# ducha-aiki/mods-light-zmq

Measured on AMD Instinct MI355X. Metric: image_pairs_per_sec_end_to_end, higher is better.
Workload: dtype f32

## Files before the change

### include/mods_hip.h

```cpp
#ifndef MODS_HIP_H
#define MODS_HIP_H

#include <stddef.h>
#include <stdint.h>

#ifdef __cplusplus
extern "C" {
#endif

#define MODS_OK 0
#define MODS_E_NODEVICE (-1)
#define MODS_E_ARG (-2)
#define MODS_E_CAPACITY (-3)
#define MODS_E_HIP (-4)

typedef struct mods_ctx mods_ctx;

typedef struct mods_hessaff_params {
  int numberOfScales;
  float initialSigma;
  float threshold;
  float edgeEigenValueRatio;
  int border;
  int maxIterations;
// ... 54 lines not shown
void *mods_ctx_stream(mods_ctx *ctx);

enum { MODS_STAGE_BLUR = 0, MODS_STAGE_RESPONSE, MODS_STAGE_RESIZE, MODS_STAGE_NMS, MODS_STAGE_LOCALIZE,
       MODS_STAGE_BAUMBERG, MODS_STAGE_SORT, MODS_STAGE_ORIENT, MODS_STAGE_DESCRIBE, MODS_STAGE_MATCH,
       MODS_STAGE_RANSAC_SCORE, MODS_STAGE_SYNTH,
       MODS_STAGE_BLUR_SMALL,
       MODS_STAGE_PYRAMID,
       MODS_STAGE_MATCH_NN1,
       MODS_STAGE_EXTRACT,
       MODS_STAGE_SIFT,
       MODS_STAGE_GUIDED,
       MODS_STAGE_MATCH_MUTUAL,
       MODS_STAGE_OVERLAP,
       MODS_STAGE_OVERLAP_AREA,
       MODS_STAGE_LOCAL_AFFINE,
       MODS_STAGE_REPROJECT_H,
       MODS_STAGE_COUNT };
int mods_ctx_timing_enable(mods_ctx *ctx, int stage_mask);
int mods_ctx_graphs(mods_ctx *ctx, int on);
long mods_ctx_graph_replays(const mods_ctx *ctx);
long mods_ctx_u8_source_calls(const mods_ctx *ctx);
int mods_ctx_u8_kernels(mods_ctx *ctx, int mask);
long mods_ctx_u8_strip_calls(const mods_ctx *ctx);
int mods_u8_strips_layout(int w, int h, unsigned *max_width, unsigned *n_strips, unsigned *pitch, size_t *image_bytes);
void mods_u8_strips_strip_of(unsigned n, unsigned *out);
int mods_u8_strips_offsets(int w, int h, unsigned *out);
int mods_u8_strips_fetch(mods_ctx *ctx, const unsigned char *img_u8_host, int n_img, int w, int h, int src_offset, unsigned char *out);
int mods_ctx_pyramid_streams(mods_ctx *ctx, int n);
int mods_ctx_timing_read(mods_ctx *ctx, int stage, double *total_ms, int *launches, double *bytes);
int mods_ctx_timing_reset(mods_ctx *ctx);

int mods_detect_hessian_affine(mods_ctx *ctx, const float *img, int w, int h, int stride,
                               const mods_hessaff_params *par, mods_affkey *out, int max_out, int *n_out);
int mods_detect_hessian_affine_dev(mods_ctx *ctx, const float *img_dev, int n_img, int w, int h, int stride,
                                   const mods_hessaff_params *par, mods_affkey *out_host, int max_out,
                                   int *n_out_host);

int mods_pyramid_octaves(mods_ctx *ctx);
int mods_pyramid_dims(mods_ctx *ctx, int octave, int *w, int *h);
int mods_pyramid_plane(mods_ctx *ctx, int img, int octave, int level, int kind, float *dst_host);
int mods_pyramid_candidates(mods_ctx *ctx, int img, mods_candidate *out, int max_out, int *n_out);
int mods_pyramid_nms_hits(mods_ctx *ctx, int img, int *out4, int max_out, int *n_out);

int mods_gauss_blur(mods_ctx *ctx, const float *src, int w, int h, float sigma, float *dst);
int mods_hessian_response(mods_ctx *ctx, const float *src, int w, int h, float norm, float *dst);
int mods_resize_half(mods_ctx *ctx, const float *src, int w, int h, float *dst, int *dw, int *dh);
// ... 450 lines not shown
```

### mods-light-zmq_amd/__init__.py

```python
import ctypes as C
import os
import subprocess

import numpy as np

PKG_DIR = os.path.dirname(os.path.abspath(__file__))
LIB_PATH = os.environ.get("MODS_LIB") or os.path.join(PKG_DIR, "libmodsgpu.so")

MODS_OK = 0
STAGES = ["blur", "response", "resize", "nms", "localize", "baumberg", "sort", "orient", "describe", "match",
          "ransac_score", "synth", "blur_small", "pyramid", "match_nn1", "extract", "sift", "guided", "match_mutual",
          "overlap", "overlap_area"]
STAGES_LATER = ["local_affine", "reproject_h"]


def stage_index(name):
    return STAGES.index(name) if name in STAGES else len(STAGES) + STAGES_LATER.index(name)


class ModsError(RuntimeError):
    pass


class HessAffParams(C.Structure):
# ... 92 lines not shown
    return out[:n.value].copy(), u6[:n.value].copy(), laf[:n.value].copy()


def _overlap(fn, dtype, lists, params, cap):
    out = np.zeros(max(cap, 1), dtype)
    n = C.c_int()
    counts = OverlapCounts()
    _check(fn(*lists, C.byref(params), _vp(out), cap, C.byref(n), C.byref(counts)))
    return out[:n.value].copy(), counts


def _mask_rows(mask):
    m = np.asarray(mask)
    if m.dtype != np.uint8 or m.ndim != 2 or m.size == 0:
        raise ValueError("a detection mask is a non-empty 2-D uint8 array")
    if m.strides[1] != 1 or m.strides[0] < m.shape[1]:
        m = np.ascontiguousarray(m)
    return m, m.strides[0]


def detection_mask_test(mask, x, y):
    m, stride = _mask_rows(mask)
    return bool(lib().mods_detection_mask_test(_vp(m), m.shape[1], m.shape[0], stride, C.c_double(x), C.c_double(y)))


def u8_strips_layout(w, h):
    lim, ns, pitch, nbytes = C.c_uint(), C.c_uint(), C.c_uint(), C.c_size_t()
    _check(lib().mods_u8_strips_layout(int(w), int(h), C.byref(lim), C.byref(ns), C.byref(pitch), C.byref(nbytes)))
    return lim.value, ns.value, pitch.value, nbytes.value


def u8_strips_strip_of(n):
    out = np.zeros(int(n), np.uint32)
    lib().mods_u8_strips_strip_of(C.c_uint(int(n)), C.c_void_p(out.ctypes.data))
    return out


def u8_strips_offsets(w, h):
    out = np.zeros((int(h) - 1, int(w) - 1), np.uint32)
    _check(lib().mods_u8_strips_offsets(int(w), int(h), C.c_void_p(out.ctypes.data)))
    return out


class ViewGeom(C.Structure):
    _fields_ = [("identity", C.c_int), ("w_rot", C.c_int), ("h_rot", C.c_int), ("w_new", C.c_int), ("h_new", C.c_int),
                ("ksize_x", C.c_int), ("ksize_y", C.c_int), ("pad", C.c_int),
# ... 298 lines not shown
        out = np.zeros(max_out, REGION_DTYPE)
        n = C.c_int()
        _check(lib().mods_orient_describe_u8(self.h, C.c_void_p(a.ctypes.data), a.shape[1], a.shape[0], a.strides[0],
                                             k.ctypes.data_as(C.c_void_p), len(k), C.byref(params), out.ctypes.data_as(C.c_void_p),
                                             max_out, C.byref(n)))
        return out[:n.value].copy()

    def regions_fetch_half(self, img=0, max_out=1 << 18):
        out = np.zeros(max_out, REGION_DTYPE)
        n = C.c_int()
        _check(lib().mods_regions_fetch_half(self.h, img, out.ctypes.data_as(C.c_void_p), max_out, C.byref(n)))
        return out[:n.value].copy()

    def detect_describe_dev(self, dev_ptr, n_img, w, h, det=None, desc=None):
        det = det or HessAffParams.default()
        desc = desc or DescribeParams.default()
        nd, nr = (C.c_int * n_img)(), (C.c_int * n_img)()
        _check(lib().mods_detect_describe_dev(self.h, C.c_void_p(dev_ptr), n_img, w, h, w, C.byref(det), C.byref(desc), nd, nr))
        return list(nd), list(nr)

    def u8_source_calls(self):
        lib().mods_ctx_u8_source_calls.restype = C.c_long
        return int(lib().mods_ctx_u8_source_calls(self.h))

    def set_u8_kernels(self, mask):
        _check(lib().mods_ctx_u8_kernels(self.h, int(mask)))

    def u8_strip_calls(self):
        lib().mods_ctx_u8_strip_calls.restype = C.c_long
        return int(lib().mods_ctx_u8_strip_calls(self.h))

    def u8_strips_fetch(self, batch_u8, src_offset=0):
        a = np.ascontiguousarray(batch_u8, np.uint8)
        n, h, w = a.shape
        _, ns, pitch, nbytes = u8_strips_layout(w, h)
        out = np.zeros(n * nbytes, np.uint8)
        _check(lib().mods_u8_strips_fetch(self.h, C.c_void_p(a.ctypes.data), n, w, h, int(src_offset), C.c_void_p(out.ctypes.data)))
        return out.reshape(n, ns, pitch // 16, 16)

    def set_match_mutual(self, mode):
        _check(lib().mods_ctx_match_mutual(self.h, int(mode)))

    def set_local_affine(self, params=None):
        _check(lib().mods_ctx_local_affine(self.h, C.byref(params) if params is not None else None))

    def local_affine_counts(self):
# ... 1180 lines not shown
```

### mods-light-zmq_amd/csrc/capi.hip

```cpp
#include "common.hpp"
#include "u8_strips.hpp"
#include "detmath.hpp"
#include "ransac_host.hpp"
#include "f_laf.hpp"
#include "h_laf.hpp"
#include "../../include/mods_degensac.h"
#include <cstdarg>
#include <memory>
#include <algorithm>
#include <cmath>
#include <mutex>
#include <vector>
#include <time.h>
#include <sys/prctl.h>

namespace mods {

static thread_local char g_err[512] = "";

void set_error(const char *fmt, ...) {
  va_list ap;
  va_start(ap, fmt);
  vsnprintf(g_err, sizeof(g_err), fmt, ap);
  va_end(ap);
// ... 421 lines not shown
    c->dd_cache.emplace_back(key, ex);
    MODS_HIP_CHECK(hipGraphLaunch(ex, c->stream));
    c->dd_replays++;
    return MODS_OK;
  }
  if (g) (void)hipGraphDestroy(g);
  (void)hipGetLastError();
  c->pyr_side = false;
  c->dd_graphs = false;
  c->omap_dirty = true;
  return dd_enqueue(c, img, n_img, w, h, stride, det, desc);
}

int mods_ctx_graphs(mods_ctx *c, int on) {
  if (!c) return MODS_E_ARG;
  c->dd_graphs = on != 0;
  if (!on) { dd_graph_drop(c); c->dd_linear.clear(); }
  mods::dev_state_changed(c);
  return MODS_OK;
}
long mods_ctx_graph_replays(const mods_ctx *c) { return c ? c->dd_replays : 0; }
long mods_ctx_u8_source_calls(const mods_ctx *c) { return c ? c->u8_source_calls : 0; }
long mods_ctx_u8_strip_calls(const mods_ctx *c) { return c ? c->u8_strip_calls : 0; }
int mods_ctx_u8_kernels(mods_ctx *c, int mask) {
  if (!c || mask > 255) { set_error("u8_kernels: bad argument"); return MODS_E_ARG; }
  c->u8_kernels = mask < 0 ? -1 : mask;
  mods::dev_state_changed(c);
  return MODS_OK;
}

static int dd_call(mods_ctx *c, const PixelSources &img, int n_img, int w, int h, int stride, const mods_hessaff_params *det,
                   const mods_describe_params *desc, int *n_detected_host, int *n_regions_host) {
  int rc;
  if ((rc = mods::dsp_check(c, desc))) return rc;
  if ((rc = dd_run(c, img, n_img, w, h, stride, det, desc))) return rc;
  int *hc = c->host_counts;
  MODS_HIP_CHECK(mods::stream_wait(c->stream));
  for (int b = 0; b < n_img; b++) {
    if (hc[b] > c->max_cand) { set_error("NMS hit list overflow: %d > %d", hc[b], c->max_cand); return MODS_E_CAPACITY; }
    if (n_detected_host) n_detected_host[b] = hc[2 * c->batch + b];
    if (hc[3 * c->batch + b] > std::min(c->max_cand, 1 << 17)) { set_error("region list overflow: %d", hc[3 * c->batch + b]); return MODS_E_CAPACITY; }
    if (n_regions_host) n_regions_host[b] = hc[3 * c->batch + b];
  }
  c->last_region_counts.assign(hc + 3 * c->batch, hc + 3 * c->batch + n_img);
  c->last_inside_counts.assign(hc + 4 * c->batch, hc + 4 * c->batch + n_img);
  if (hc[5 * c->batch]) {
// ... 778 lines not shown
```

### mods-light-zmq_amd/csrc/common.hpp

```cpp
#pragma once
#include <hip/hip_runtime.h>
#include <atomic>
#include <chrono>
#include <cmath>
#include <cstdint>
#include <cstdio>
#include <cstring>
#include <string>
#include <vector>
#include "../../include/mods_hip.h"
#include "buffer.hpp"
#include "pixel_sources.hpp"
#include "detection_mask.hpp"

namespace mods {

void set_error(const char *fmt, ...);

#define MODS_HIP_CHECK(expr)                                                              \
  do {                                                                                    \
    hipError_t _e = (expr);                                                               \
    if (_e != hipSuccess) {                                                               \
      mods::set_error("%s failed: %s (%s:%d)", #expr, hipGetErrorString(_e), __FILE__, __LINE__); \
      return MODS_E_HIP;                                                                  \
// ... 163 lines not shown
  mods::Buf<int> cand_count;
  mods::Buf<mods_affkey> keys_dev;
  mods::Buf<unsigned long long> sort_keys;
  mods::Buf<int> sort_idx;
  mods::Buf<int> rank_dev;
  mods::Buf<unsigned long long> nms_mask;
  mods::PinnedBuf<int> host_counts;
  mods::Buf<unsigned char> u8_stage_dev;
  mods::Buf<unsigned char> u8_strip_dev;
  long u8_strip_calls = 0;
  int u8_kernels = -1;
  long u8_source_calls = 0;
  mods::Buf<unsigned char> clahe_lut;
  bool clahe_on = false;
  mods_clahe_params clahe_par = {0.0, 0, 0};
  mods::PinnedBuf<char> pin_arena;
  mods_hessaff_params par;
  int reg_number_eff = -1;
  int last_w = 0, last_h = 0, last_n_img = 0;
  const float *last_img_dev = nullptr; int last_stride = 0;
  mods::Buf<float> desc_tables_dev;
  mods::Buf<int> desc_err_dev;
  int desc_ori_ps = 0, desc_ps = 0;
  mods::Buf<char> ori_dev;
  mods::Buf<char> ori_multi_dev;
  mods::Buf<mods_region> regions_dev;
  mods::Buf<mods_region> regions_half_dev;
  bool have_half = false;
  mods::Buf<int> region_count;
  mods::Buf<int> inside_count;
  std::vector<int> last_inside_counts;
  mods::Buf<float> desc_scratch;
  int dsp_scales = 0;
  double dsp_start = 0, dsp_end = 0;
  mods::Buf<double> dsp_acc;
  int blur_table_ps = 0;
  mods::Buf<float> blur_table_dev;
  mods_descriptor_fn ext_fn = nullptr;
  void *ext_user = nullptr;
  double ext_mr = 0;
  int ext_ps = 0;
  mods_descriptor_fn shape_fn = nullptr, ori_fn = nullptr;
  void *shape_user = nullptr, *ori_user = nullptr;
  double shape_mr = 0, ori_mr = 0;
  int shape_ps = 0, ori_ps = 0;
  mods_net *shape_net = nullptr, *ori_net = nullptr, *ext_net = nullptr;
// ... 157 lines not shown
__host__ __device__ inline int la_len(int n, int max_n) { return n < 0 || n > max_n ? 0 : n; }
int la_check(const mods_local_affine_params *p, LaConst *k);
int la_reserve(mods_ctx *c, int n_jobs, int grid_n);
int la_filter_dev(mods_ctx *c, const LaJob *jobs, int n_jobs, int grid_n, const LaConst &k, const int **diag_counters = nullptr,
                  const int **diag_slots = nullptr, int *diag_stride = nullptr);
struct TentList;
int local_affine_prefilter(mods_ctx *c, const mods_pair_params *par, TentList *list, bool deduped);
static_assert(LA_MAX_JOBS >= kCountSlots - 1, "every pair of a batch has its slots in la_count");
int launch_fast_sqrt_selftest(mods_ctx *ctx, unsigned long long *out5_host);
int launch_blur_table(mods_ctx *ctx, int ps);
bool ransac_profile_on();
int ransac_profile_mode();

int describe_run(mods_ctx *ctx, const PixelSources &img, int n_img, int w, int h, const mods_describe_params *par);
int u8_to_f32_launch(mods_ctx *c, const unsigned char *src, int n_img, int w, int h, int stride, float *dst, bool strips = false);
int u8_sources_launch(mods_ctx *c, const unsigned char *src, int n_img, int w, int h, int stride, bool twin, PixelSources *img);
int u8_stage_ensure(mods_ctx *c);
int describe_run_view(mods_ctx *ctx, const PixelSources &img, int n_img, int w, int h, const mods_describe_params *par, const double *H,
                      int orig_w, int orig_h, mods_region *det_copy_dev);
bool view_region_frame(const double *H, int w, int h, int orig_w, int orig_h, DetGateFrame *frame);
int describe_configure(mods_ctx *ctx, const mods_describe_params *par);
int launch_dominant_angle_test(mods_ctx *ctx, const float *patch_dev, int ps, double th, float *out_dev);
int launch_sift_patch_test(mods_ctx *ctx, const float *patch_dev, int ps, int root, double max_bin, uint8_t *out_dev);
int launch_sift_pooled_test(mods_ctx *ctx, const float *patches_dev, int K, int ps, int root, int half, int photo, double max_bin,
                            uint8_t *out_dev);
int dsp_check(mods_ctx *ctx, const mods_describe_params *par);

inline bool has_hooks(const mods_ctx *c) { return c->ext_fn || c->shape_fn || c->ori_fn; }
inline bool has_nets(const mods_ctx *c) { return c->ext_net || c->shape_net || c->ori_net; }
int net_run_to_host(mods_ctx *ctx, mods_net *net, const float *patches_dev, int n, int quantise_u8, float *out_host);

int pair_gpu_stage(mods_ctx *c, const float *img_dev, int w, int h, int stride, const mods_pair_params *par, mods_pair_result *res,
                   TentList *list);
int pairs_gpu_stage(mods_ctx *c, const void *const *img, const int *kinds, int n_pairs, int w, int h, const mods_pair_params *par,
                    mods_pair_result *const *res, TentList *const *lists, const unsigned char *const *masks = nullptr);
int pair_verify_stage(int device, const mods_pair_params *par, mods_pair_result *res, TentList *list, double *matches_out,
                      int max_matches, int w, int h);

}

extern "C" {
int mods_match_copy_out(mods_ctx *c, int n, mods_tentative *tent, double *u6, double *laf);
int mods_match_fetch_internal(mods_ctx *c, mods_tentative *out, double *u6_out, double *laf_out, int max_out, int *n_out);
int mods_ransac_warmup(int device, int len);
int mods_ctx_warmup(mods_ctx *c, int n_img, int w, int h, const mods_pair_params *par);
}
// ... 1 lines not shown
```

### mods-light-zmq_amd/csrc/describe.hip

```cpp
#include "describe_common.hpp"
#include "detmath.hpp"
#include "device_util.hpp"

namespace mods {

struct OriOut { double a11, a12, a21, a22; int alive; int pad; };

__device__ unsigned char g_ori_bin[2048];
__global__ __launch_bounds__(256) void ori_bin_table_kernel() {
  const float PIf = 3.14159265358979323846f;
  const int bins = 36;
  const int e = blockIdx.x * 256 + threadIdx.x;
  const float ori = atan2_lut_case(e >> 8, g_atan_lut[e & 255]);
  g_ori_bin[e] = (unsigned char)(int)(bins * (ori / PIf + 1.0f) / 2.0f);
}

__device__ __forceinline__ float peak_angle(const float *s_hist, int b) {
  const int bins = 36;
  const float PIf = 3.14159265358979323846f;
  const int a = b == 0 ? bins - 1 : b - 1, c = b == bins - 1 ? 0 : b + 1;
  const float ha = s_hist[a], hb = s_hist[b], hc = s_hist[c];
  const float pp = (ha - hc) / (ha - 2.0f * hb + hc) / 2.0f;
  return 2.0f * PIf * (b + 0.5f + pp) / bins - PIf;
}
// ... 421 lines not shown
      !(par->desc_patchSize & 1)) { set_error("unsupported patch sizes (ori %d, desc %d)", par->ori_patchSize, par->desc_patchSize); return MODS_E_ARG; }
  if (!ctx->desc_tables_dev) {
    MODS_HIP_CHECK(mods::reserve_group(ctx->desc_tables_dev, kTabSift + (sizeof(SiftTab) + sizeof(float) - 1) / sizeof(float), ctx->desc_err_dev, 1));
    MODS_HIP_CHECK(hipMemsetAsync(ctx->desc_err_dev, 0, sizeof(int), ctx->stream));
  }
  if (ctx->desc_ori_ps != par->ori_patchSize || ctx->desc_ps != par->desc_patchSize) {
    std::vector<float> m1((size_t)64 * 64, 0.f), m2((size_t)64 * 64, 0.f);
    circular_gauss_mask_host(par->ori_patchSize, par->ori_patchSize / 3.0f, m1.data());
    circular_gauss_mask_host(par->desc_patchSize, 0.f, m2.data());
    SiftTab tab;
    build_sift_tab(par->desc_patchSize, &tab);
    mods::dev_state_changed(ctx);
    MODS_HIP_CHECK(mods::stream_wait(ctx->stream));
    MODS_HIP_CHECK(mods::copy_wait(ctx->stream, ctx->desc_tables_dev, m1.data(), sizeof(float) * 4096, hipMemcpyHostToDevice));
    MODS_HIP_CHECK(mods::copy_wait(ctx->stream, ctx->desc_tables_dev + kTabDescMask, m2.data(), sizeof(float) * 4096, hipMemcpyHostToDevice));
    {
      const int ps = par->ori_patchSize;
      std::vector<float> vm((size_t)64 * 64, 0.f);
      for (int p = 0; p < ps * (ps - 2); p++) { const int c = p % ps; vm[p] = (c >= 1 && c < ps - 1) ? m1[p + ps] : 0.f; }
      MODS_HIP_CHECK(mods::copy_wait(ctx->stream, ctx->desc_tables_dev + kTabVoteMask, vm.data(), sizeof(float) * 4096, hipMemcpyHostToDevice));
    }
    MODS_HIP_CHECK(mods::copy_wait(ctx->stream, ctx->desc_tables_dev + kTabSift, &tab, sizeof(SiftTab), hipMemcpyHostToDevice));
    ctx->desc_ori_ps = par->ori_patchSize; ctx->desc_ps = par->desc_patchSize;
  }
  return MODS_OK;
}

int describe_run(mods_ctx *ctx, const PixelSources &img, int n_img, int w, int h, const mods_describe_params *par) {
  return describe_run_view(ctx, img, n_img, w, h, par, nullptr, 0, 0, nullptr);
}

static int external_describe(mods_ctx *ctx, int n_img, const DescConst &k) {
  const int pp = k.desc_ps * k.desc_ps;
  std::vector<int> counts(n_img);
  MODS_HIP_CHECK(hipMemcpyAsync(counts.data(), ctx->region_count, sizeof(int) * n_img, hipMemcpyDeviceToHost, ctx->stream));
  MODS_HIP_CHECK(mods::stream_wait(ctx->stream));
  std::vector<float> patches, out;
  std::vector<uint8_t> desc;
  for (int b = 0; b < n_img; b++) {
    const int n = std::min(counts[b], k.reg_cap);
    if (n <= 0) continue;
    out.assign((size_t)n * 128, 0.f); desc.resize((size_t)n * 128);
    if (ctx->ext_net) {
      const int rc = net_run_to_host(ctx, ctx->ext_net, ctx->desc_scratch + (size_t)b * k.reg_cap * pp, n, ctx->ext_q8, out.data());
      if (rc) return rc;
    } else {
// ... 316 lines not shown
```

### mods-light-zmq_amd/csrc/sift.hip

```cpp
#include "describe_common.hpp"
#include "detmath.hpp"
#include "device_util.hpp"

namespace mods {

constexpr int SMALL_CAP = 80;
#ifndef EXTRACT_T_LO
#define EXTRACT_T_LO 48
#endif
#ifndef EXTRACT_T_MID
#define EXTRACT_T_MID 64
#endif
#ifndef ES_MINB
#define ES_MINB 5
#endif

__device__ __forceinline__ double *lds_doubles(float *base, const void *p) {
  const int off = (int)((const float *)p - base);
  return (double *)(base + ((off + 1) & ~1));
}

struct RegionGeom {
  int P2;
  float scale;
// ... 1055 lines not shown
      sift_tail(s_vec, s_sq, s_red, k.root != 0, k.max_bin, o + (size_t)b * img_stride + (size_t)ri * reg_stride, half != 0);
    }
  }
}

constexpr int SW_R = 8;
constexpr int SW_G = 68;
constexpr int SW_CW = 18;
constexpr int S2_MAX_IMG = 64;
constexpr int S2_WAVES = 12;
constexpr int S2_BINS = 1024;
__device__ __forceinline__ int s2_bin(int g, int br, int bc) { return (g >> 2) * 64 + br * 16 + (g & 3) * 4 + bc; }
__device__ __forceinline__ int s2_vec(int g, int i) { return (i & 7) * 128 + s2_bin(g, i >> 5, (i >> 3) & 3); }

__host__ __device__ constexpr int s2_row_slots(int ps) { return SW_R * ps + SW_CW + 2 > SW_R * SW_G / 2 ? SW_R * ps + SW_CW + 2 : SW_R * SW_G / 2; }
static size_t sift_wave2_wave_bytes(int ps) {
  return sizeof(double) * S2_BINS + sizeof(float2) * (size_t)s2_row_slots(ps) + sizeof(float) * 3 * SW_R;
}
static size_t sift_wave2_lds_bytes(int ps) {
  const size_t ppa = ((size_t)ps * ps + 7) & ~(size_t)7;
  return sizeof(float) * 2048 + sizeof(float) * (4 * ps + 4) + sizeof(int) * 72 + sizeof(unsigned short) * ppa + S2_WAVES * sift_wave2_wave_bytes(ps) + 64;
}

template <int NC, bool POOL = false>
__global__ __launch_bounds__(64 * S2_WAVES, 3) void sift_wave2_kernel(DescConst k, const float *__restrict__ patches, mods_region *__restrict__ reg_all,
                                                                        const int *__restrict__ reg_count, const float *__restrict__ mask,
                                                                        const SiftTab *__restrict__ tab, int n_img, int *__restrict__ next_unit,
                                                                        double *__restrict__ pool, int pool_first) {
  extern __shared__ __attribute__((aligned(16))) float smem[];
  const int ps = k.desc_ps, pp = ps * ps, ppa = (pp + 7) & ~7;
  const int tid = threadIdx.x, lane = tid & 63, wv = tid >> 6;
  float *s_ot = smem;
  float *s_w = s_ot + 2048;
  int *s_pref = (int *)(s_w + 4 * ps + 4);
  unsigned short *s_midx = (unsigned short *)(s_pref + 72);
  unsigned char *wbase = (unsigned char *)(s_midx + ppa) + (size_t)wv * (sizeof(double) * S2_BINS + sizeof(float2) * s2_row_slots(ps) + sizeof(float) * 3 * SW_R);
  double *acc = (double *)wbase;
  float2 *pxrow = (float2 *)(acc + S2_BINS);
  float *s_mean = (float *)(pxrow + s2_row_slots(ps)), *s_fac = s_mean + SW_R;
  int *s_flag = (int *)(s_fac + SW_R);
  float *g = (float *)pxrow;
  const int rowf = SW_R * ps;

  const double M_PI_DOUBLED = 6.28318530718;
  sift_tables(tab, ps, s_w);
  for (int i = tid; i < 2048; i += 64 * S2_WAVES) {
    const float ori = atan2_lut_case(i >> 8, g_atan_lut[i & 255]);
    s_ot[i] = (float)(8.0f * ((double)ori + M_PI_DOUBLED) / M_PI_DOUBLED);
  }
  if (tid < 64) {
    int c = 0;
    for (int base = 0; base < pp; base += 64) {
      const int p = base + tid;
      const bool m = p < pp && mask[p] > 0;
      const unsigned long long bm = __ballot(m);
      if (m) s_midx[c + __popcll(bm & ((1ull << tid) - 1ull))] = (unsigned short)p;
      c += __popcll(bm);
    }
    if (tid == 0) s_pref[68] = c;
  }
  if (tid == 64) {
    int cum = 0;
    for (int b = 0; b < n_img; b++) { s_pref[b] = cum; int n = reg_count[b]; if (n > k.reg_cap) n = k.reg_cap; cum += (n + SW_R - 1) / SW_R; }
    s_pref[n_img] = cum;
  }
  __syncthreads();
  const int n_mask = s_pref[68];
  const int total_units = s_pref[n_img];
  const float o_zero = (float)(8.0f * ((double)0.f + M_PI_DOUBLED) / M_PI_DOUBLED);

  const int hr = lane >> 3, hsel = (lane >> 2) & 1, hbc = lane & 3;
  int clo = ps;
  for (int i = ps - 1; i >= 0; i--) if (s_w[hbc * ps + i] > 0) clo = i;
  float wcw[NC];
#pragma unroll
  for (int q = 0; q < NC; q++) wcw[q] = (clo + q < ps) ? s_w[hbc * ps + clo + q] : 0.f;
  constexpr int RL = 6;
  int s_rr[RL], s_c[RL];
#pragma unroll
  for (int u = 0; u < RL; u++) { const int e = lane + 64 * u; s_rr[u] = e < rowf ? e / ps : SW_R - 1; s_c[u] = e < rowf ? e - (e / ps) * ps : 0; }

#ifdef SIFT_PROF
  unsigned long long pt[6] = {0, 0, 0, 0, 0, 0}, pl = __builtin_amdgcn_s_memtime();
  int pn = 0;
#define S2PROF(i) { const unsigned long long t_ = __builtin_amdgcn_s_memtime(); pt[i] += t_ - pl; pl = t_; }
#else
#define S2PROF(i)
#endif
  for (;;) {
    int unit = 0;
    if (lane == 0) unit = atomicAdd(next_unit, 1);
    unit = __builtin_amdgcn_readfirstlane(unit);
    if (unit >= total_units) break;
    int b = 0;
    while (b + 1 < n_img && s_pref[b + 1] <= unit) b++;
    const int ri0 = (unit - s_pref[b]) * SW_R;
    mods_region *reg = reg_all + (size_t)b * k.max_reg;
    int n = reg_count[b];
    if (n > k.reg_cap) n = k.reg_cap;
    const float *pbase = patches + (size_t)b * k.reg_cap * pp;
    auto patch_of = [&](int rr) { return pbase + (size_t)min(ri0 + rr, n - 1) * pp; };
    wave_sync();
    S2PROF(0)
// ... 30 lines not shown
            for (; q + 15 < cnt; q += 16) {
              const float4 a0 = *(const float4 *)(gl + q), a1 = *(const float4 *)(gl + q + 4), a2 = *(const float4 *)(gl + q + 8), a3 = *(const float4 *)(gl + q + 12);
              sum += a0.x; sum += a0.y; sum += a0.z; sum += a0.w; sum += a1.x; sum += a1.y; sum += a1.z; sum += a1.w;
              sum += a2.x; sum += a2.y; sum += a2.z; sum += a2.w; sum += a3.x; sum += a3.y; sum += a3.z; sum += a3.w;
            }
            for (; q + 3 < cnt; q += 4) {
              const float4 a = *(const float4 *)(gl + q);
              sum += a.x; sum += a.y; sum += a.z; sum += a.w;
            }
            for (; q < cnt; q++) sum += gl[q];
          }
        }
        if (lane < SW_R) {
          if (pass == 0) s_mean[lane] = sum / (float)n_mask;
          else {
            const float var = sqrtf(sum / (float)n_mask);
            if (!((double)var < 0.0001)) { s_flag[lane] = 1; s_fac[lane] = 50.0f / var; }
          }
        }
        wave_sync();
      }
    }
    wave_sync();
    S2PROF(1)
    unsigned sbyte[RL], cbyte[RL];
    float sm[RL], sf[RL];
    unsigned nflag = 0;
#pragma unroll
    for (int u = 0; u < RL; u++) {
      sbyte[u] = ((unsigned)min(ri0 + s_rr[u], n - 1) * (unsigned)pp + (unsigned)s_c[u]) * 4u;
      cbyte[u] = (unsigned)s_c[u] * 4u;
      sm[u] = s_mean[s_rr[u]]; sf[u] = s_fac[s_rr[u]];
      nflag |= (s_flag[s_rr[u]] ? 1u : 0u) << u;
    }
    auto fetch_row = [&](int r, float *dst) {
      const char *rowp = (const char *)(pbase + r * ps);
#pragma unroll
      for (int u = 0; u < RL; u++) dst[u] = *(const float *)(rowp + sbyte[u]);
    };
    auto norm_row = [&](const float *raw, float *dst) {
#pragma unroll
      for (int u = 0; u < RL; u++) {
        const float t = __builtin_amdgcn_fmed3f(128 + sf[u] * (raw[u] - sm[u]), 0.f, 255.f);
        dst[u] = ((nflag >> u) & 1) ? t : raw[u];
      }
    };
    auto fetch_mask = [&](int r, float *dst) {
      const char *mrowp = (const char *)(mask + r * ps);
#pragma unroll
      for (int u = 0; u < RL; u++) dst[u] = *(const float *)(mrowp + cbyte[u]);
    };
    float nm[RL], n0[RL], np[RL], ra[RL], rb[RL], mcur[RL];
    fetch_row(0, ra); norm_row(ra, n0);
    fetch_row(min(1, ps - 1), ra); norm_row(ra, np);
    fetch_row(min(2, ps - 1), ra);
    fetch_row(min(3, ps - 1), rb);
    fetch_mask(0, mcur);
#pragma unroll
    for (int u = 0; u < RL; u++) nm[u] = n0[u];
#pragma unroll 1
    for (int r = 0; r < ps; r++) {
      {
        const unsigned last_col = 4u * (unsigned)(ps - 1);
#pragma unroll
        for (int u = 0; u < RL; u++) {
          const int e = lane + 64 * u;
          float right = lane_down1(n0[u]), left = lane_up1(n0[u]);
          if (u + 1 < RL) { const float nx = __int_as_float(__builtin_amdgcn_readlane(__float_as_int(n0[u + 1 < RL ? u + 1 : u]), 0)); right = lane == 63 ? nx : right; }
          if (u > 0) { const float pl = __int_as_float(__builtin_amdgcn_readlane(__float_as_int(n0[u > 0 ? u - 1 : u]), 63)); left = lane == 0 ? pl : left; }
          const float xa = cbyte[u] < last_col ? right : n0[u];
          const float xb = cbyte[u] > 0u ? left : n0[u];
          const float xgrad = xa - xb, ygrad = np[u] - nm[u];
          const float grad = fast_sqrtf_any(xgrad * xgrad + ygrad * ygrad);
          const AtanSel as = atan2_lut_sel(ygrad, xgrad);
          const float ot = s_ot[as.oct * 256 + as.idx];
          const float o = as.zero ? o_zero : ot;
          if (e < rowf) pxrow[e] = make_float2(mcur[u] * grad, o);
        }
      }
      fetch_mask(min(r + 1, ps - 1), mcur);
      wave_sync();
      S2PROF(2)
      {
        const int rb8 = hsel ? tab->bin1[r] : tab->bin0[r];
        const float wrr = hsel ? tab->w1[r] : tab->w0[r];
        if (wrr > 0) {
          double *abin = acc + s2_bin(hr, rb8 >> 3, hbc);
          const float2 *px = pxrow + hr * ps + clo;
#pragma unroll
          for (int q0 = 0; q0 < NC; q0 += NC / 2) {
            float2 pv[NC / 2];
#pragma unroll
            for (int q = 0; q < NC / 2; q++) pv[q] = px[q0 + q];
#pragma unroll
            for (int q = 0; q < NC / 2; q++) {
              const float val = wrr * (wcw[q0 + q] * pv[q].x);
              const bool on = val > 0;
              const int bo0 = (int)pv[q].y;
              const float y = pv[q].y - bo0;
              const float c0 = on ? val * (1.0f - y) : 0.f, c1 = on ? val * y : 0.f;
              __hip_atomic_fetch_add(abin + (bo0 & 7) * 128, (double)c0, __ATOMIC_RELAXED, __HIP_MEMORY_SCOPE_WAVEFRONT);
              __hip_atomic_fetch_add(abin + ((bo0 + 1) & 7) * 128, (double)c1, __ATOMIC_RELAXED, __HIP_MEMORY_SCOPE_WAVEFRONT);
            }
          }
        }
      }
      wave_sync();
      S2PROF(3)
#pragma unroll
      for (int u = 0; u < RL; u++) { nm[u] = n0[u]; n0[u] = np[u]; }
      norm_row(ra, np);
#pragma unroll
      for (int u = 0; u < RL; u++) ra[u] = rb[u];
      fetch_row(min(r + 4, ps - 1), rb);
      S2PROF(4)
    }
    wave_sync();
    if constexpr (POOL) {
      const int rr = lane >> 3;
      if (ri0 + rr < n) {
        double *dst = pool + ((size_t)b * k.reg_cap + ri0 + rr) * 128;
        for (int i = lane & 7; i < 128; i += 8) {
          const double x = acc[s2_vec(rr, i)];
          dst[i] = pool_first ? x : dst[i] + x;
        }
      }
      continue;
    }
    double *tmp = (double *)pxrow;
    unsigned long long redo = ~0ull;
    for (int pass = 0; pass < 2; pass++) {
      if (lane < SW_R && ((redo >> (8 * lane)) & 1)) {
        double len = 0.0;
#pragma unroll 1
        for (int i = 0; i < 128; i += 8) {
          double x[8];
#pragma unroll
// ... 80 lines not shown
                                                              uint8_t *out) {
  extern __shared__ __attribute__((aligned(16))) float smem[];
  SiftLds L(smem, ps);
  sift_tables(tab, ps, L.w);
  for (int i = threadIdx.x; i < 256; i += 256) L.lut[i] = g_atan_lut[i];
  for (int p = threadIdx.x; p < ps * ps; p += 256) L.patch[p] = patch[p];
  __syncthreads();
  sift_from_patch(L.patch, mask, L.w, L.lut, ps, root != 0, max_bin, L.px, L.bo, L.vec, L.red, out);
}

static int sift_col_span(int ps) {
  int span = 0;
  const float step = 5.0f / (float)(2 * (ps >> 1));
  for (int bc = 0; bc < 4; bc++) {
    int lo = ps, hi = -1;
    for (int i = 0; i < ps; i++) {
      const float x = step * i; const int xi = (int)x; const float w1 = x - xi, w0 = 1.0f - w1;
      const bool on = (xi - 1 == bc && w0 > 0) || (xi == bc && w1 > 0);
      if (on) { lo = std::min(lo, i); hi = i; }
    }
    if (hi >= lo) span = std::max(span, hi - lo + 1);
  }
  return span;
}

int launch_extract_and_sift(mods_ctx *ctx, const PixelSources &img, int n_img, DescConst k, const float *dmask, const SiftTab *tab, bool run_sift) {
  StageScope ts(ctx, MODS_STAGE_DESCRIBE);
  const int ps = k.desc_ps, ps2 = 2 * ps, pp = ps * ps;
  const size_t patch_elems = (size_t)n_img * k.reg_cap * pp;
  const int max_big = 1 << 17, max_items = 1 << 20;
  const int small_cap_items = n_img * k.reg_cap;
  const size_t book_elems = (sizeof(BigLists) + sizeof(BigRegion) * max_big + 3 * sizeof(int2) * max_items + 3 * sizeof(int) * (size_t)small_cap_items + 15) / 4;
  const unsigned long long area_units = std::max<unsigned long long>(1, ((unsigned long long)k.w * k.h + (1ull << 21) - 1) >> 21);
  const unsigned long long pool_elems = std::max<unsigned long long>(256ull << 20, (unsigned long long)n_img * area_units * (64ull << 20));
  const size_t need = patch_elems + book_elems + pool_elems;
  MODS_HIP_CHECK(mods::reserve_pool(ctx, ctx->desc_scratch, need, need));
  float *patches = ctx->desc_scratch;
  BigLists *bl = (BigLists *)(ctx->desc_scratch + patch_elems);
  BigRegion *bregs = (BigRegion *)(bl + 1);
  int2 *sitems = (int2 *)(bregs + max_big);
  int2 *ritems = sitems + max_items;
  int2 *fitems = ritems + max_items;
  int *small_items = (int *)(fitems + max_items);
  float *pool = ctx->desc_scratch + patch_elems + book_elems;
  MODS_HIP_CHECK(hipMemsetAsync(bl, 0, sizeof(BigLists), ctx->stream));
  { const int trc = launch_blur_table(ctx, ps); if (trc) return trc; }
// ... 19 lines not shown
                           (const float *)ctx->blur_table_dev);
      });
    }
  }
  const size_t ldsH = sizeof(float) * (k.tap_cap + 4 * ps2) + 32;
  hipLaunchKernelGGL(big_setup_kernel, dim3(1024), dim3(256), ldsH, ctx->stream, k, bl, bregs, max_big, pool, ctx->desc_err_dev);
  with_pixel_source(ctx->u8_kernels, img, U8K_BIG_FUSED, [&](auto *px) {
    hipLaunchKernelGGL(big_fused_kernel<PixelOf<decltype(px)>>, dim3(8192), dim3(256), BIG_FUSE_KB * 1024, ctx->stream, px, k, bl, bregs, fitems,
                       max_items, ctx->regions_dev, pool, ctx->desc_err_dev);
  });
  with_pixel_source(ctx->u8_kernels, img, U8K_BIG_SAMPLE, [&](auto *px) {
    hipLaunchKernelGGL(big_sample_kernel<PixelOf<decltype(px)>>, dim3(4096), dim3(256), 0, ctx->stream, px, k, bl, bregs, sitems, max_items,
                       ctx->regions_dev, pool, ctx->desc_err_dev);
  });
  hipLaunchKernelGGL(big_rowpass_kernel, dim3(4096), dim3(256), 0, ctx->stream, k, bl, bregs, ritems, max_items, pool,
                     ctx->desc_err_dev);
  hipLaunchKernelGGL(big_colres_kernel, dim3(4096), dim3(256), 0, ctx->stream, k, bl, bregs, max_big, pool, patches, ctx->desc_err_dev);
  }
  StageScope ts_sift(ctx, MODS_STAGE_SIFT);
  if (run_sift && ps > 45)
    hipLaunchKernelGGL(sift_kernel, dim3(2048, n_img), dim3(256), sift_lds_bytes(ps), ctx->stream, k, patches, ctx->regions_dev,
                       ctx->region_count, dmask, tab);
  else if (run_sift) {
    static DynLdsOnce once16, once18;
    MODS_HIP_CHECK(dyn_lds_once(once16, (const void *)sift_wave2_kernel<16>, 160 * 1024, ctx->device));
    MODS_HIP_CHECK(dyn_lds_once(once18, (const void *)sift_wave2_kernel<SW_CW>, 160 * 1024, ctx->device));
    const int span = sift_col_span(ps);
    for (int b0 = 0; b0 < n_img; b0 += S2_MAX_IMG) {
      const int nb = std::min(S2_MAX_IMG, n_img - b0);
      if (b0) MODS_HIP_CHECK(hipMemsetAsync(&bl->sift_next, 0, sizeof(int), ctx->stream));
      const float *pch = patches + (size_t)b0 * k.reg_cap * pp;
      mods_region *regs = ctx->regions_dev + (size_t)b0 * k.max_reg;
      if (span <= 16)
        hipLaunchKernelGGL(sift_wave2_kernel<16>, dim3(ctx->n_cu), dim3(64 * S2_WAVES), sift_wave2_lds_bytes(ps), ctx->stream, k, pch,
                           regs, ctx->region_count + b0, dmask, tab, nb, &bl->sift_next, (double *)nullptr, 0);
      else
        hipLaunchKernelGGL(sift_wave2_kernel<SW_CW>, dim3(ctx->n_cu), dim3(64 * S2_WAVES), sift_wave2_lds_bytes(ps), ctx->stream, k, pch,
                           regs, ctx->region_count + b0, dmask, tab, nb, &bl->sift_next, (double *)nullptr, 0);
    }
  }
  MODS_HIP_CHECK(hipGetLastError());
  return MODS_OK;
}

int launch_half_sift(mods_ctx *ctx, int n_img, DescConst k, const float *dmask, const SiftTab *tab) {
  StageScope ts(ctx, MODS_STAGE_DESCRIBE);
  MODS_HIP_CHECK(ctx->regions_half_dev.reserve((size_t)ctx->max_cand * ctx->batch));
  MODS_HIP_CHECK(hipMemcpyAsync(ctx->regions_half_dev, ctx->regions_dev, sizeof(mods_region) * (size_t)ctx->max_cand * n_img,
                                hipMemcpyDeviceToDevice, ctx->stream));
  k.half_desc = 1;
  const int ps = k.desc_ps;
  const float *patches = ctx->desc_scratch;
  hipLaunchKernelGGL(sift_kernel, dim3(2048, n_img), dim3(256), sift_lds_bytes(ps), ctx->stream, k, patches, ctx->regions_half_dev,
                     ctx->region_count, dmask, tab);
  MODS_HIP_CHECK(hipGetLastError());
  return MODS_OK;
}

static int dsp_accumulate(mods_ctx *ctx, const float *patches, double *acc, const int *reg_count, int *next_unit, int n_img, DescConst k,
                          const float *dmask, const SiftTab *tab, bool first) {
  const int ps = k.desc_ps, pp = ps * ps;
  if (ps > 45) {
    hipLaunchKernelGGL(dsp_accumulate_kernel, dim3(2048, n_img), dim3(256), sift_lds_bytes(ps), ctx->stream, k, patches, acc, reg_count, dmask,
                       tab, first ? 1 : 0);
    MODS_HIP_CHECK(hipGetLastError());
    return MODS_OK;
  }
  static DynLdsOnce once16, once18;
  MODS_HIP_CHECK(dyn_lds_once(once16, (const void *)sift_wave2_kernel<16, true>, 160 * 1024, ctx->device));
  MODS_HIP_CHECK(dyn_lds_once(once18, (const void *)sift_wave2_kernel<SW_CW, true>, 160 * 1024, ctx->device));
  const int span = sift_col_span(ps);
  for (int b0 = 0; b0 < n_img; b0 += S2_MAX_IMG) {
    const int nb = std::min(S2_MAX_IMG, n_img - b0);
    if (b0) MODS_HIP_CHECK(hipMemsetAsync(next_unit, 0, sizeof(int), ctx->stream));
    const float *pch = patches + (size_t)b0 * k.reg_cap * pp;
    double *pool = acc + (size_t)b0 * k.reg_cap * 128;
    if (span <= 16)
      hipLaunchKernelGGL((sift_wave2_kernel<16, true>), dim3(ctx->n_cu), dim3(64 * S2_WAVES), sift_wave2_lds_bytes(ps), ctx->stream, k, pch,
                         (mods_region *)nullptr, reg_count + b0, dmask, tab, nb, next_unit, pool, first ? 1 : 0);
    else
      hipLaunchKernelGGL((sift_wave2_kernel<SW_CW, true>), dim3(ctx->n_cu), dim3(64 * S2_WAVES), sift_wave2_lds_bytes(ps), ctx->stream, k, pch,
                         (mods_region *)nullptr, reg_count + b0, dmask, tab, nb, next_unit, pool, first ? 1 : 0);
  }
  MODS_HIP_CHECK(hipGetLastError());
  return MODS_OK;
}

int launch_dsp_accumulate(mods_ctx *ctx, int n_img, DescConst k, const float *dmask, const SiftTab *tab, bool first) {
  StageScope ts(ctx, MODS_STAGE_DESCRIBE);
  StageScope ts_sift(ctx, MODS_STAGE_SIFT);
  BigLists *bl = (BigLists *)(ctx->desc_scratch + (size_t)n_img * k.reg_cap * k.desc_ps * k.desc_ps);
  return dsp_accumulate(ctx, ctx->desc_scratch, ctx->dsp_acc, ctx->region_count, &bl->sift_next, n_img, k, dmask, tab, first);
}

int launch_dsp_finish(mods_ctx *ctx, int n_img, DescConst k, bool want_half) {
  StageScope ts(ctx, MODS_STAGE_DESCRIBE);
  StageScope ts_sift(ctx, MODS_STAGE_SIFT);
  uint8_t *out_half = nullptr;
  if (want_half) {
    MODS_HIP_CHECK(ctx->regions_half_dev.reserve((size_t)ctx->max_cand * ctx->batch));
    MODS_HIP_CHECK(hipMemcpyAsync(ctx->regions_half_dev, ctx->regions_dev, sizeof(mods_region) * (size_t)ctx->max_cand * n_img,
                                  hipMemcpyDeviceToDevice, ctx->stream));
    out_half = (uint8_t *)ctx->regions_half_dev.get() + offsetof(mods_region, desc);
  }
  hipLaunchKernelGGL(dsp_finish_kernel, dim3(4096, n_img), dim3(128), 0, ctx->stream, k, (const double *)ctx->dsp_acc.get(),
// ... 35 lines not shown
```

Measured before the change: 1061.

## Skip masked rows and drop dead last column in wave SIFT kernel

Adds a five-slot variant of the wave-level SIFT kernel, chosen when the circular Gaussian mask zeroes the last patch column. In that case each lane handles five row slots instead of six, and the boundary pixel is fetched separately. The kernel also builds a per-row liveness bitmask from the mask and skips the gradient and histogram work, plus the wave syncs, for rows whose mask is all zero. This cuts per-row ALU, LDS and barrier work, at the cost of extra code paths, a one-column store offset and one more template instantiation. It also adds launch counters.

```diff
diff --git a/include/mods_hip.h b/include/mods_hip.h
--- a/include/mods_hip.h
+++ b/include/mods_hip.h
@@ -100,6 +100,8 @@
 long mods_ctx_u8_source_calls(const mods_ctx *ctx);
 int mods_ctx_u8_kernels(mods_ctx *ctx, int mask);
 long mods_ctx_u8_strip_calls(const mods_ctx *ctx);
+long mods_ctx_sift_slot_launches(const mods_ctx *ctx, int five);
+int mods_sift_row_slots(int desc_patchSize);
 int mods_u8_strips_layout(int w, int h, unsigned *max_width, unsigned *n_strips, unsigned *pitch, size_t *image_bytes);
 void mods_u8_strips_strip_of(unsigned n, unsigned *out);
 int mods_u8_strips_offsets(int w, int h, unsigned *out);
diff --git a/mods-light-zmq_amd/__init__.py b/mods-light-zmq_amd/__init__.py
--- a/mods-light-zmq_amd/__init__.py
+++ b/mods-light-zmq_amd/__init__.py
@@ -138,6 +138,10 @@
 def detection_mask_test(mask, x, y):
     m, stride = _mask_rows(mask)
     return bool(lib().mods_detection_mask_test(_vp(m), m.shape[1], m.shape[0], stride, C.c_double(x), C.c_double(y)))
+
+
+def sift_row_slots(desc_patch_size):
+    return int(lib().mods_sift_row_slots(int(desc_patch_size)))
 
 
 def u8_strips_layout(w, h):
@@ -482,6 +486,10 @@
     def u8_source_calls(self):
         lib().mods_ctx_u8_source_calls.restype = C.c_long
         return int(lib().mods_ctx_u8_source_calls(self.h))
+
+    def sift_slot_launches(self, five):
+        lib().mods_ctx_sift_slot_launches.restype = C.c_long
+        return int(lib().mods_ctx_sift_slot_launches(self.h, int(bool(five))))
 
     def set_u8_kernels(self, mask):
         _check(lib().mods_ctx_u8_kernels(self.h, int(mask)))
diff --git a/mods-light-zmq_amd/csrc/capi.hip b/mods-light-zmq_amd/csrc/capi.hip
--- a/mods-light-zmq_amd/csrc/capi.hip
+++ b/mods-light-zmq_amd/csrc/capi.hip
@@ -467,6 +467,13 @@
 long mods_ctx_graph_replays(const mods_ctx *c) { return c ? c->dd_replays : 0; }
 long mods_ctx_u8_source_calls(const mods_ctx *c) { return c ? c->u8_source_calls : 0; }
 long mods_ctx_u8_strip_calls(const mods_ctx *c) { return c ? c->u8_strip_calls : 0; }
+long mods_ctx_sift_slot_launches(const mods_ctx *c, int five) { return c ? c->sift_slot_launches[five ? 1 : 0] : 0; }
+int mods_sift_row_slots(int ps) {
+  if (ps < 3 || ps > 63) return 0;
+  std::vector<float> m((size_t)64 * 64, 0.f);
+  mods::circular_gauss_mask_host(ps, 0.f, m.data());
+  return mods::sift_five_slots(m.data(), ps) ? 5 : 6;
+}
 int mods_ctx_u8_kernels(mods_ctx *c, int mask) {
   if (!c || mask > 255) { set_error("u8_kernels: bad argument"); return MODS_E_ARG; }
   c->u8_kernels = mask < 0 ? -1 : mask;
diff --git a/mods-light-zmq_amd/csrc/common.hpp b/mods-light-zmq_amd/csrc/common.hpp
--- a/mods-light-zmq_amd/csrc/common.hpp
+++ b/mods-light-zmq_amd/csrc/common.hpp
@@ -209,6 +209,8 @@
   mods::Buf<float> desc_tables_dev;
   mods::Buf<int> desc_err_dev;
   int desc_ori_ps = 0, desc_ps = 0;
+  int sift_five_ps = 0;
+  long sift_slot_launches[2] = {0, 0};
   mods::Buf<char> ori_dev;
   mods::Buf<char> ori_multi_dev;
   mods::Buf<mods_region> regions_dev;
@@ -412,6 +414,7 @@
 int describe_configure(mods_ctx *ctx, const mods_describe_params *par);
 int launch_dominant_angle_test(mods_ctx *ctx, const float *patch_dev, int ps, double th, float *out_dev);
 int launch_sift_patch_test(mods_ctx *ctx, const float *patch_dev, int ps, int root, double max_bin, uint8_t *out_dev);
+bool sift_five_slots(const float *mask, int ps);
 int launch_sift_pooled_test(mods_ctx *ctx, const float *patches_dev, int K, int ps, int root, int half, int photo, double max_bin,
                             uint8_t *out_dev);
 int dsp_check(mods_ctx *ctx, const mods_describe_params *par);
diff --git a/mods-light-zmq_amd/csrc/describe.hip b/mods-light-zmq_amd/csrc/describe.hip
--- a/mods-light-zmq_amd/csrc/describe.hip
+++ b/mods-light-zmq_amd/csrc/describe.hip
@@ -467,6 +467,7 @@
     }
     MODS_HIP_CHECK(mods::copy_wait(ctx->stream, ctx->desc_tables_dev + kTabSift, &tab, sizeof(SiftTab), hipMemcpyHostToDevice));
     ctx->desc_ori_ps = par->ori_patchSize; ctx->desc_ps = par->desc_patchSize;
+    ctx->sift_five_ps = sift_five_slots(m2.data(), par->desc_patchSize) ? par->desc_patchSize : 0;
   }
   return MODS_OK;
 }
diff --git a/mods-light-zmq_amd/csrc/sift.hip b/mods-light-zmq_amd/csrc/sift.hip
--- a/mods-light-zmq_amd/csrc/sift.hip
+++ b/mods-light-zmq_amd/csrc/sift.hip
@@ -1101,7 +1101,7 @@
   return sizeof(float) * 2048 + sizeof(float) * (4 * ps + 4) + sizeof(int) * 72 + sizeof(unsigned short) * ppa + S2_WAVES * sift_wave2_wave_bytes(ps) + 64;
 }
 
-template <int NC, bool POOL = false>
+template <int NC, bool POOL = false, bool C5 = false>
 __global__ __launch_bounds__(64 * S2_WAVES, 3) void sift_wave2_kernel(DescConst k, const float *__restrict__ patches, mods_region *__restrict__ reg_all,
                                                                         const int *__restrict__ reg_count, const float *__restrict__ mask,
                                                                         const SiftTab *__restrict__ tab, int n_img, int *__restrict__ next_unit,
@@ -1119,7 +1119,6 @@
   float *s_mean = (float *)(pxrow + s2_row_slots(ps)), *s_fac = s_mean + SW_R;
   int *s_flag = (int *)(s_fac + SW_R);
   float *g = (float *)pxrow;
-  const int rowf = SW_R * ps;
 
   const double M_PI_DOUBLED = 6.28318530718;
   sift_tables(tab, ps, s_w);
@@ -1138,6 +1137,13 @@
     }
     if (tid == 0) s_pref[68] = c;
   }
+  if (tid >= 128 && tid < 192) {
+    const int r = tid - 128;
+    bool live = false;
+    if (r < ps) for (int c = 0; c < ps; c++) live = live || mask[r * ps + c] > 0;
+    const unsigned long long bm = __ballot(live);
+    if (tid == 128) { s_pref[69] = (int)(unsigned)bm; s_pref[70] = (int)(unsigned)(bm >> 32); }
+  }
   if (tid == 64) {
     int cum = 0;
     for (int b = 0; b < n_img; b++) { s_pref[b] = cum; int n = reg_count[b]; if (n > k.reg_cap) n = k.reg_cap; cum += (n + SW_R - 1) / SW_R; }
@@ -1146,6 +1152,8 @@
   __syncthreads();
   const int n_mask = s_pref[68];
   const int total_units = s_pref[n_img];
+  const unsigned long long rowlive = ((unsigned long long)(unsigned)__builtin_amdgcn_readfirstlane(s_pref[70]) << 32) |
+                                     (unsigned)__builtin_amdgcn_readfirstlane(s_pref[69]);
   const float o_zero = (float)(8.0f * ((double)0.f + M_PI_DOUBLED) / M_PI_DOUBLED);
 
   const int hr = lane >> 3, hsel = (lane >> 2) & 1, hbc = lane & 3;
@@ -1154,10 +1162,16 @@
   float wcw[NC];
 #pragma unroll
   for (int q = 0; q < NC; q++) wcw[q] = (clo + q < ps) ? s_w[hbc * ps + clo + q] : 0.f;
-  constexpr int RL = 6;
+  constexpr int RL = C5 ? 5 : 6;
+  const int pw = C5 ? ps - 1 : ps, rowl = SW_R * pw;
   int s_rr[RL], s_c[RL];
-#pragma unroll
-  for (int u = 0; u < RL; u++) { const int e = lane + 64 * u; s_rr[u] = e < rowf ? e / ps : SW_R - 1; s_c[u] = e < rowf ? e - (e / ps) * ps : 0; }
+  int xu = -1;
+#pragma unroll
+  for (int u = 0; u < RL; u++) {
+    const int e = lane + 64 * u;
+    s_rr[u] = e < rowl ? e / pw : SW_R - 1; s_c[u] = e < rowl ? e - (e / pw) * pw : 0;
+    if (C5 && e < rowl && s_c[u] == pw - 1) xu = u;
+  }
 
 #ifdef SIFT_PROF
   unsigned long long pt[6] = {0, 0, 0, 0, 0, 0}, pl = __builtin_amdgcn_s_memtime();
@@ -1234,6 +1248,7 @@
       }
     }
     wave_sync();
+    if (C5 && lane < SW_R) pxrow[lane * ps + ps - 1] = make_float2(0.f, o_zero);
     S2PROF(1)
     unsigned sbyte[RL], cbyte[RL];
     float sm[RL], sf[RL];
@@ -1245,17 +1260,30 @@
       sm[u] = s_mean[s_rr[u]]; sf[u] = s_fac[s_rr[u]];
       nflag |= (s_flag[s_rr[u]] ? 1u : 0u) << u;
     }
-    auto fetch_row = [&](int r, float *dst) {
+    unsigned xbyte = 0;
+    float xsm = 0.f, xsf = 0.f;
+    bool xfl = false;
+    if (C5) {
+#pragma unroll
+      for (int u = 0; u < RL; u++)
+        if (u == xu) { xbyte = sbyte[u] + 4u; xsm = sm[u]; xsf = sf[u]; xfl = (nflag >> u) & 1; }
+    }
+    auto fetch_row = [&](int r, float *dst, float &xdst) {
       const char *rowp = (const char *)(pbase + r * ps);
 #pragma unroll
       for (int u = 0; u < RL; u++) dst[u] = *(const float *)(rowp + sbyte[u]);
+      if (C5 && xu >= 0) xdst = *(const float *)(rowp + xbyte);
     };
-    auto norm_row = [&](const float *raw, float *dst) {
+    auto norm_row = [&](const float *raw, float *dst, float xraw, float &xdst) {
 #pragma unroll
       for (int u = 0; u < RL; u++) {
         const float t = __builtin_amdgcn_fmed3f(128 + sf[u] * (raw[u] - sm[u]), 0.f, 255.f);
         dst[u] = ((nflag >> u) & 1) ? t : raw[u];
       }
+      if (C5) {
+        const float t = __builtin_amdgcn_fmed3f(128 + xsf * (xraw - xsm), 0.f, 255.f);
+        xdst = xfl ? t : xraw;
+      }
     };
     auto fetch_mask = [&](int r, float *dst) {
       const char *mrowp = (const char *)(mask + r * ps);
@@ -1263,16 +1291,18 @@
       for (int u = 0; u < RL; u++) dst[u] = *(const float *)(mrowp + cbyte[u]);
     };
     float nm[RL], n0[RL], np[RL], ra[RL], rb[RL], mcur[RL];
-    fetch_row(0, ra); norm_row(ra, n0);
-    fetch_row(min(1, ps - 1), ra); norm_row(ra, np);
-    fetch_row(min(2, ps - 1), ra);
-    fetch_row(min(3, ps - 1), rb);
+    float x0 = 0.f, xp = 0.f, xa = 0.f, xb = 0.f;
+    fetch_row(0, ra, xa); norm_row(ra, n0, xa, x0);
+    fetch_row(min(1, ps - 1), ra, xa); norm_row(ra, np, xa, xp);
+    fetch_row(min(2, ps - 1), ra, xa);
+    fetch_row(min(3, ps - 1), rb, xb);
     fetch_mask(0, mcur);
 #pragma unroll
     for (int u = 0; u < RL; u++) nm[u] = n0[u];
 #pragma unroll 1
     for (int r = 0; r < ps; r++) {
-      {
+      const bool live = (rowlive >> r) & 1ull;
+      if (live) {
         const unsigned last_col = 4u * (unsigned)(ps - 1);
 #pragma unroll
         for (int u = 0; u < RL; u++) {
@@ -1280,20 +1310,20 @@
           float right = lane_down1(n0[u]), left = lane_up1(n0[u]);
           if (u + 1 < RL) { const float nx = __int_as_float(__builtin_amdgcn_readlane(__float_as_int(n0[u + 1 < RL ? u + 1 : u]), 0)); right = lane == 63 ? nx : right; }
           if (u > 0) { const float pl = __int_as_float(__builtin_amdgcn_readlane(__float_as_int(n0[u > 0 ? u - 1 : u]), 63)); left = lane == 0 ? pl : left; }
-          const float xa = cbyte[u] < last_col ? right : n0[u];
-          const float xb = cbyte[u] > 0u ? left : n0[u];
-          const float xgrad = xa - xb, ygrad = np[u] - nm[u];
+          const float gr = C5 ? (u == xu ? x0 : right) : (cbyte[u] < last_col ? right : n0[u]);
+          const float gl = cbyte[u] > 0u ? left : n0[u];
+          const float xgrad = gr - gl, ygrad = np[u] - nm[u];
           const float grad = fast_sqrtf_any(xgrad * xgrad + ygrad * ygrad);
           const AtanSel as = atan2_lut_sel(ygrad, xgrad);
           const float ot = s_ot[as.oct * 256 + as.idx];
           const float o = as.zero ? o_zero : ot;
-          if (e < rowf) pxrow[e] = make_float2(mcur[u] * grad, o);
+          if (e < rowl) pxrow[C5 ? e + s_rr[u] : e] = make_float2(mcur[u] * grad, o);
         }
       }
       fetch_mask(min(r + 1, ps - 1), mcur);
-      wave_sync();
-      S2PROF(2)
-      {
+      if (live) {
+        wave_sync();
+        S2PROF(2)
         const int rb8 = hsel ? tab->bin1[r] : tab->bin0[r];
         const float wrr = hsel ? tab->w1[r] : tab->w0[r];
         if (wrr > 0) {
@@ -1316,15 +1346,17 @@
             }
           }
         }
-      }
-      wave_sync();
-      S2PROF(3)
+        wave_sync();
+        S2PROF(3)
+      }
 #pragma unroll
       for (int u = 0; u < RL; u++) { nm[u] = n0[u]; n0[u] = np[u]; }
-      norm_row(ra, np);
+      x0 = xp;
+      norm_row(ra, np, xa, xp);
 #pragma unroll
       for (int u = 0; u < RL; u++) ra[u] = rb[u];
-      fetch_row(min(r + 4, ps - 1), rb);
+      xa = xb;
+      fetch_row(min(r + 4, ps - 1), rb, xb);
       S2PROF(4)
     }
     wave_sync();
@@ -1451,6 +1483,34 @@
     if (hi >= lo) span = std::max(span, hi - lo + 1);
   }
   return span;
+}
+
+bool sift_five_slots(const float *mask, int ps) {
+  const int pw = ps - 1;
+  if (ps < 3 || ps > 45 || SW_R * pw > 5 * 64) return false;
+  for (int r = 0; r < ps; r++)
+    if (mask[r * ps + ps - 1] != 0) return false;
+  for (int lane = 0; lane < 64; lane++) {
+    int held = 0;
+    for (int e = lane; e < SW_R * pw; e += 64) held += e % pw == pw - 1;
+    if (held > 1) return false;
+  }
+  return true;
+}
+
+template <int NC, bool POOL, bool C5>
+static int sift_wave2_launch(mods_ctx *ctx, DescConst k, const float *pch, mods_region *regs, const int *reg_count, const float *dmask,
+                             const SiftTab *tab, int nb, int *next_unit, double *pool, int first) {
+  static DynLdsOnce once;
+  MODS_HIP_CHECK(dyn_lds_once(once, (const void *)sift_wave2_kernel<NC, POOL, C5>, 160 * 1024, ctx->device));
+  hipLaunchKernelGGL((sift_wave2_kernel<NC, POOL, C5>), dim3(ctx->n_cu), dim3(64 * S2_WAVES), sift_wave2_lds_bytes(k.desc_ps), ctx->stream, k,
+                     pch, regs, reg_count, dmask, tab, nb, next_unit, pool, first);
+  ctx->sift_slot_launches[C5 ? 1 : 0]++;
+  return MODS_OK;
+}
+template <int NC, bool POOL, class... Args> static int sift_wave2_launch_form(mods_ctx *ctx, DescConst k, Args... args) {
+  if (ctx->sift_five_ps == k.desc_ps) return sift_wave2_launch<NC, POOL, true>(ctx, k, args...);
+  return sift_wave2_launch<NC, POOL, false>(ctx, k, args...);
 }
 
 int launch_extract_and_sift(mods_ctx *ctx, const PixelSources &img, int n_img, DescConst k, const float *dmask, const SiftTab *tab, bool run_sift) {
@@ -1516,21 +1576,18 @@
     hipLaunchKernelGGL(sift_kernel, dim3(2048, n_img), dim3(256), sift_lds_bytes(ps), ctx->stream, k, patches, ctx->regions_dev,
                        ctx->region_count, dmask, tab);
   else if (run_sift) {
-    static DynLdsOnce once16, once18;
-    MODS_HIP_CHECK(dyn_lds_once(once16, (const void *)sift_wave2_kernel<16>, 160 * 1024, ctx->device));
-    MODS_HIP_CHECK(dyn_lds_once(once18, (const void *)sift_wave2_kernel<SW_CW>, 160 * 1024, ctx->device));
     const int span = sift_col_span(ps);
     for (int b0 = 0; b0 < n_img; b0 += S2_MAX_IMG) {
       const int nb = std::min(S2_MAX_IMG, n_img - b0);
       if (b0) MODS_HIP_CHECK(hipMemsetAsync(&bl->sift_next, 0, sizeof(int), ctx->stream));
       const float *pch = patches + (size_t)b0 * k.reg_cap * pp;
       mods_region *regs = ctx->regions_dev + (size_t)b0 * k.max_reg;
+      int rc;
       if (span <= 16)
-        hipLaunchKernelGGL(sift_wave2_kernel<16>, dim3(ctx->n_cu), dim3(64 * S2_WAVES), sift_wave2_lds_bytes(ps), ctx->stream, k, pch,
-                           regs, ctx->region_count + b0, dmask, tab, nb, &bl->sift_next, (double *)nullptr, 0);
+        rc = sift_wave2_launch_form<16, false>(ctx, k, pch, regs, (const int *)(ctx->region_count + b0), dmask, tab, nb, &bl->sift_next, (double *)nullptr, 0);
       else
-        hipLaunchKernelGGL(sift_wave2_kernel<SW_CW>, dim3(ctx->n_cu), dim3(64 * S2_WAVES), sift_wave2_lds_bytes(ps), ctx->stream, k, pch,
-                           regs, ctx->region_count + b0, dmask, tab, nb, &bl->sift_next, (double *)nullptr, 0);
+        rc = sift_wave2_launch_form<SW_CW, false>(ctx, k, pch, regs, (const int *)(ctx->region_count + b0), dmask, tab, nb, &bl->sift_next, (double *)nullptr, 0);
+      if (rc) return rc;
     }
   }
   MODS_HIP_CHECK(hipGetLastError());
@@ -1560,21 +1617,18 @@
     MODS_HIP_CHECK(hipGetLastError());
     return MODS_OK;
   }
-  static DynLdsOnce once16, once18;
-  MODS_HIP_CHECK(dyn_lds_once(once16, (const void *)sift_wave2_kernel<16, true>, 160 * 1024, ctx->device));
-  MODS_HIP_CHECK(dyn_lds_once(once18, (const void *)sift_wave2_kernel<SW_CW, true>, 160 * 1024, ctx->device));
   const int span = sift_col_span(ps);
   for (int b0 = 0; b0 < n_img; b0 += S2_MAX_IMG) {
     const int nb = std::min(S2_MAX_IMG, n_img - b0);
     if (b0) MODS_HIP_CHECK(hipMemsetAsync(next_unit, 0, sizeof(int), ctx->stream));
     const float *pch = patches + (size_t)b0 * k.reg_cap * pp;
     double *pool = acc + (size_t)b0 * k.reg_cap * 128;
+    int rc;
     if (span <= 16)
-      hipLaunchKernelGGL((sift_wave2_kernel<16, true>), dim3(ctx->n_cu), dim3(64 * S2_WAVES), sift_wave2_lds_bytes(ps), ctx->stream, k, pch,
-                         (mods_region *)nullptr, reg_count + b0, dmask, tab, nb, next_unit, pool, first ? 1 : 0);
+      rc = sift_wave2_launch_form<16, true>(ctx, k, pch, (mods_region *)nullptr, reg_count + b0, dmask, tab, nb, next_unit, pool, first ? 1 : 0);
     else
-      hipLaunchKernelGGL((sift_wave2_kernel<SW_CW, true>), dim3(ctx->n_cu), dim3(64 * S2_WAVES), sift_wave2_lds_bytes(ps), ctx->stream, k, pch,
-                         (mods_region *)nullptr, reg_count + b0, dmask, tab, nb, next_unit, pool, first ? 1 : 0);
+      rc = sift_wave2_launch_form<SW_CW, true>(ctx, k, pch, (mods_region *)nullptr, reg_count + b0, dmask, tab, nb, next_unit, pool, first ? 1 : 0);
+    if (rc) return rc;
   }
   MODS_HIP_CHECK(hipGetLastError());
   return MODS_OK;
```

After: 1072, median of 5. 1.0% higher.
